# Aleph-Alpha/magma

Measured on NVIDIA H100. Metric: image-caption samples/sec (fwd+bwd), higher is better.
Workload: dtype bf16

## Files before the change

magma_b200/csrc/gemm.cu:

```cuda
#include <mutex>
#include <stdlib.h>

#include "gemm_common.cuh"

namespace mb200 {

template <int BN, bool A_MN, bool B_MN>
__global__ void __launch_bounds__(kThreads, 1)
gemm_wgmma_kernel(const __grid_constant__ CUtensorMap tmA, const __grid_constant__ CUtensorMap tmB,
                  const __grid_constant__ GemmKernelParams p) {
  using C_ = Cfg<BN>;
  constexpr int kStages = C_::kStages;

  extern __shared__ uint8_t smem_raw[];
  uint8_t* smem = reinterpret_cast<uint8_t*>((reinterpret_cast<uintptr_t>(smem_raw) + 1023) & ~uintptr_t(1023));
  uint8_t* smem_a = smem;
  uint8_t* smem_b = smem + kStages * C_::kABytes;
  float* epi_stage = reinterpret_cast<float*>(smem + kStages * C_::kStageBytes);
  uint64_t* full_bar = reinterpret_cast<uint64_t*>(smem + kStages * C_::kStageBytes + kEpiBytes);
  uint64_t* empty_bar = full_bar + kStages;

  const int wg = threadIdx.x >> 7;
  const int num_kb = (p.K + BK - 1) / BK;
  const int items = p.total_tiles * p.split_k;

  pdl_trigger();
  if (threadIdx.x == 0) {
    tma_prefetch_desc(&tmA);
    tma_prefetch_desc(&tmB);
    for (int s = 0; s < kStages; ++s) {
      mbar_init(&full_bar[s], 1);
      mbar_init(&empty_bar[s], 2);
    }
    mbar_fence_init();
  }
  __syncthreads();
  pdl_wait();

  if (wg == 0) {
    setmaxnreg_dec<40>();
    if (threadIdx.x == 0) {
      int stage = 0;
      uint32_t phase = 0;
      for (int w = blockIdx.x; w < items; w += gridDim.x) {
        const int t = w / p.split_k, ks = w - t * p.split_k;
        const int kb0 = ks * p.kb_per_split, kb1 = min(num_kb, kb0 + p.kb_per_split);
        const int tpb = p.tiles_m * p.tiles_n;
        const int z = t / tpb;
        const int r = t - z * tpb;
        const int m_blk = r % p.tiles_m;
        const int n_blk = r / p.tiles_m;
        const int z0 = z % p.nb0, z1 = z / p.nb0;
        for (int kb = kb0; kb < kb1; ++kb) {
          mbar_wait(&empty_bar[stage], phase ^ 1);
          mbar_expect_tx(&full_bar[stage], (uint32_t)C_::kStageBytes);
          uint8_t* sa = smem_a + stage * C_::kABytes;
          uint8_t* sb = smem_b + stage * C_::kBBytes;
          const int kc = kb * BK;
          if constexpr (A_MN) {
#pragma unroll
            for (int i = 0; i < BM / 64; ++i)
              tma_load_4d(sa + i * 8192, &tmA, &full_bar[stage], m_blk * BM + i * 64, kc, z0, z1);
          } else {
            tma_load_4d(sa, &tmA, &full_bar[stage], kc, m_blk * BM, z0, z1);
          }
          if constexpr (B_MN) {
#pragma unroll
            for (int i = 0; i < BN / 64; ++i)
              tma_load_4d(sb + i * 8192, &tmB, &full_bar[stage], n_blk * BN + i * 64, kc, z0, z1);
          } else {
            tma_load_4d(sb, &tmB, &full_bar[stage], kc, n_blk * BN, z0, z1);
          }
          if (++stage == kStages) {
            stage = 0;
            phase ^= 1;
          }
        }
      }
    }
  } else {
    setmaxnreg_inc<232>();
    const int cw = wg - 1;
    const bool leader = (threadIdx.x & 127) == 0;
    constexpr uint32_t b_lbo = B_MN ? 8192u : 0u;
    constexpr uint32_t a_kadv = A_MN ? 2048u : 32u, b_kadv = B_MN ? 2048u : 32u;
    const uint32_t a_off = (uint32_t)cw * 8192u;
    int stage = 0;
    uint32_t phase = 0;
    float acc[BN / 2];
    for (int w = blockIdx.x; w < items; w += gridDim.x) {
      const int t = w / p.split_k, ks = w - t * p.split_k;
      const int kb0 = ks * p.kb_per_split, kb1 = min(num_kb, kb0 + p.kb_per_split);
      const int tpb = p.tiles_m * p.tiles_n;
      const int z = t / tpb;
      const int r = t - z * tpb;
      const int m_blk = r % p.tiles_m;
      const int n_blk = r / p.tiles_m;
      const int z0 = z % p.nb0, z1 = z / p.nb0;
      int prev = -1;
      for (int kb = kb0; kb < kb1; ++kb) {
        mbar_wait(&full_bar[stage], phase);
        const uint32_t sa = smem_u32(smem_a + stage * C_::kABytes) + a_off;
        const uint32_t sb = smem_u32(smem_b + stage * C_::kBBytes);
        wgmma_fence();
#pragma unroll
        for (int k = 0; k < BK / WG_K; ++k) {
          const uint64_t da = make_smem_desc(sa + k * a_kadv, 0u, 1024);
          const uint64_t db = make_smem_desc(sb + k * b_kadv, b_lbo, 1024);
          wgmma_bf16<BN, A_MN ? 1 : 0, B_MN ? 1 : 0>(acc, da, db, (kb > kb0 || k > 0) ? 1u : 0u);
        }
        wgmma_commit();
        wgmma_wait<1>();
        if (prev >= 0 && leader) mbar_arrive(&empty_bar[prev]);
        prev = stage;
        if (++stage == kStages) {
          stage = 0;
          phase ^= 1;
        }
      }
      wgmma_wait<0>();
      if (prev >= 0 && leader) mbar_arrive(&empty_bar[prev]);
      const long long boff = (long long)z0 * p.c_bs0 + (long long)z1 * p.c_bs1;
      epi_tile<BN>(p, acc, epi_stage + cw * 64 * kEpiCols, 1 + cw, boff, m_blk * BM + cw * 64, n_blk * BN, ks);
    }
  }
}

__global__ void splitk_finalize_kernel(const GemmKernelParams p) {
  pdl_trigger();
  pdl_wait();
  const int ncol4 = (p.N + 3) >> 2;
  const long long total = (long long)p.M * ncol4;
  for (long long i = blockIdx.x * (long long)blockDim.x + threadIdx.x; i < total; i += (long long)gridDim.x * blockDim.x) {
    const int row = (int)(i / ncol4);
    const int col = (int)(i - (long long)row * ncol4) * 4;
    float v[4] = {0.f, 0.f, 0.f, 0.f};
    for (int ks = 0; ks < p.split_k; ++ks) {
      const float4 w4 = *reinterpret_cast<const float4*>(p.splitk_ws + ((long long)ks * p.M + row) * p.ld_ws + col);
      v[0] += w4.x;
      v[1] += w4.y;
      v[2] += w4.z;
      v[3] += w4.w;
    }
    epi_store4(p, 0, row, col, v);
  }
}

typedef CUresult (*PFN_encodeTiled)(CUtensorMap*, CUtensorMapDataType, cuuint32_t, void*, const cuuint64_t*,
                                    const cuuint64_t*, const cuuint32_t*, const cuuint32_t*, CUtensorMapInterleave,
                                    CUtensorMapSwizzle, CUtensorMapL2promotion, CUtensorMapFloatOOBfill);

static PFN_encodeTiled get_encode_fn() {
  static PFN_encodeTiled fn = nullptr;
  static std::once_flag once;
  std::call_once(once, [] {
    void* p = nullptr;
    cudaDriverEntryPointQueryResult qres;
    if (cudaGetDriverEntryPoint("cuTensorMapEncodeTiled", &p, cudaEnableDefault, &qres) == cudaSuccess &&
        qres == cudaDriverEntryPointSuccess)
      fn = reinterpret_cast<PFN_encodeTiled>(p);
  });
  return fn;
}

int make_operand_map(CUtensorMap* out, const mb200_operand& op, int rows, int K, int nb0, int nb1,
                            int box_rows) {
  PFN_encodeTiled enc = get_encode_fn();
  MB_REQUIRE(enc != nullptr, MB200_E_CUDA, "cuTensorMapEncodeTiled entry point unavailable");
  MB_REQUIRE((reinterpret_cast<uintptr_t>(op.ptr) & 15) == 0, MB200_E_ALIGN, "gemm operand pointer not 16B aligned");
  MB_REQUIRE(op.ld % 8 == 0, MB200_E_ALIGN, "gemm operand ld (%lld) must be a multiple of 8 elements",
             (long long)op.ld);
  MB_REQUIRE((nb0 == 1 || op.bs0 % 8 == 0) && (nb1 == 1 || op.bs1 % 8 == 0), MB200_E_ALIGN,
             "gemm operand batch strides must be multiples of 8 elements");
  cuuint64_t dims[4];
  cuuint64_t strides[3];
  cuuint32_t box[4];
  cuuint32_t estr[4] = {1, 1, 1, 1};
  if (!op.mn_major) {
    dims[0] = (cuuint64_t)K;
    dims[1] = (cuuint64_t)rows;
    box[0] = BK;
    box[1] = (cuuint32_t)box_rows;
  } else {
    dims[0] = (cuuint64_t)rows;
    dims[1] = (cuuint64_t)K;
    box[0] = 64;
    box[1] = BK;
  }
  dims[2] = (cuuint64_t)nb0;
  dims[3] = (cuuint64_t)nb1;
  box[2] = 1;
  box[3] = 1;
  strides[0] = (cuuint64_t)op.ld * 2;
  strides[1] = (cuuint64_t)(nb0 > 1 ? op.bs0 : op.ld) * 2;
  strides[2] = (cuuint64_t)(nb1 > 1 ? op.bs1 : op.ld) * 2;
  CUresult r = enc(out, CU_TENSOR_MAP_DATA_TYPE_BFLOAT16, 4, const_cast<void*>(op.ptr), dims, strides, box, estr,
                   CU_TENSOR_MAP_INTERLEAVE_NONE, CU_TENSOR_MAP_SWIZZLE_128B, CU_TENSOR_MAP_L2_PROMOTION_L2_256B,
                   CU_TENSOR_MAP_FLOAT_OOB_FILL_NONE);
  MB_REQUIRE(r == CUDA_SUCCESS, MB200_E_CUDA,
             "cuTensorMapEncodeTiled failed (%d): dims=(%llu,%llu,%llu,%llu) strides=(%llu,%llu,%llu) box=(%u,%u)",
             (int)r, (unsigned long long)dims[0], (unsigned long long)dims[1], (unsigned long long)dims[2],
             (unsigned long long)dims[3], (unsigned long long)strides[0], (unsigned long long)strides[1],
             (unsigned long long)strides[2], box[0], box[1]);
  return 0;
}

template <int BN, bool A_MN, bool B_MN>
static int launch_gemm(const CUtensorMap& tmA, const CUtensorMap& tmB, const GemmKernelParams& kp,
                       cudaStream_t stream) {
  auto kern = gemm_wgmma_kernel<BN, A_MN, B_MN>;
  static bool attr_set = false;
  if (!attr_set) {
    MB_CUDA(cudaFuncSetAttribute(kern, cudaFuncAttributeMaxDynamicSharedMemorySize, Cfg<BN>::kSmemBytes));
    attr_set = true;
  }
  const long long items = (long long)kp.total_tiles * kp.split_k;
  int grid = items < gemm_sms() ? (int)items : gemm_sms();
  {
    const double nb = (double)kp.total_tiles / ((double)kp.tiles_m * kp.tiles_n);
    const double flops = 2.0 * kp.M * (double)kp.N * kp.K * nb;
    const double bytes = nb * (2.0 * ((double)kp.M * kp.K + (double)kp.N * kp.K) + (kp.c_f32 ? 4.0 : 2.0) * kp.M * kp.N);
    GemmProfScope prof(stream, flops, bytes);
    MB_CUDA(launch_pdl(kern, dim3(grid), dim3(kThreads), Cfg<BN>::kSmemBytes, stream, tmA, tmB, kp));
  }
  count_launch();
  MB_CUDA(cudaGetLastError());
  return 0;
}

template <int BN>
static int dispatch_major(bool a_mn, bool b_mn, const CUtensorMap& tmA, const CUtensorMap& tmB,
                          const GemmKernelParams& kp, cudaStream_t s) {
  if (!a_mn && !b_mn) return launch_gemm<BN, false, false>(tmA, tmB, kp, s);
  if (!a_mn && b_mn) return launch_gemm<BN, false, true>(tmA, tmB, kp, s);
  if (a_mn && !b_mn) return launch_gemm<BN, true, false>(tmA, tmB, kp, s);
  return launch_gemm<BN, true, true>(tmA, tmB, kp, s);
}

static int dispatch_bn(int bn, bool a_mn, bool b_mn, const CUtensorMap& tmA, const CUtensorMap& tmB,
                       const GemmKernelParams& kp, cudaStream_t s) {
  switch (bn) {
    case 64: return dispatch_major<64>(a_mn, b_mn, tmA, tmB, kp, s);
    case 128: return dispatch_major<128>(a_mn, b_mn, tmA, tmB, kp, s);
    default: return dispatch_major<256>(a_mn, b_mn, tmA, tmB, kp, s);
  }
}

static int pick_bn(int M, int N, int batches) {
  if (N <= 64) return 64;
  const int tiles_m = (M + BM - 1) / BM;
  const int sms = num_sms();
  double best = 1e300;
  int best_bn = 256;
  const int cands[3] = {256, 128, 64};
  const double tile_cost[3] = {1.0, 0.55, 0.3};
  for (int i = 0; i < 3; ++i) {
    const int bn = cands[i];
    if (bn > 64 && N <= bn / 2) continue;
    const long long t = (long long)tiles_m * ((N + bn - 1) / bn) * batches;
    const long long waves = (t + sms - 1) / sms;
    const double cost = (double)waves * tile_cost[i];
    if (cost < best - 1e-12) {
      best = cost;
      best_bn = bn;
    }
  }
  return best_bn;
}

struct SmallPlan {
  int bn, split;
};
static SmallPlan plan_small_m(int N, int K, int M, size_t ws_bytes) {
  const int sms = num_sms();
  const int num_kb = (K + BK - 1) / BK;
  const double kHbmRate = 3.35e12, kItem = 4e-6, kFinalize = 4e-6;
  SmallPlan best{64, 1};
  double best_t = 1e300;
  const int cands[3] = {256, 128, 64};
  for (int i = 0; i < 3; ++i) {
    const int bn = cands[i];
    if (bn > 64 && N <= bn / 2) continue;
    const int tiles = (N + bn - 1) / bn;
    for (int split = 1; split <= 16; ++split) {
      if (split > 1) {
        if (num_kb / split < 8) break;
        if ((size_t)split * M * ((N + 3) / 4 * 4) * sizeof(float) > ws_bytes) break;
      }
      const int kb_per = (num_kb + split - 1) / split;
      const int eff_split = (num_kb + kb_per - 1) / kb_per;
      const long long items = (long long)tiles * eff_split;
      const long long waves = (items + sms - 1) / sms;
      const double active = (double)(items < sms ? items : sms);
      const double sm_rate = bn == 64 ? 40e9 : 50e9;
      const double rate = sm_rate < kHbmRate / active ? sm_rate : kHbmRate / active;
      const double t = kItem + waves * ((double)kb_per * bn * BK * 2 / rate) + (eff_split > 1 ? kFinalize : 0.0);
      if (t < best_t - 1e-12) {
        best_t = t;
        best = SmallPlan{bn, eff_split};
      }
    }
  }
  return best;
}

int gemm_impl(const mb200_gemm_args* a, cudaStream_t stream) {
  MB_REQUIRE(a != nullptr, MB200_E_ARG, "null gemm args");
  MB_REQUIRE(a->M > 0 && a->N > 0 && a->K > 0 && a->nb0 > 0 && a->nb1 > 0, MB200_E_SHAPE,
             "gemm: bad shape M=%d N=%d K=%d nb=(%d,%d)", a->M, a->N, a->K, a->nb0, a->nb1);
  MB_REQUIRE(a->c_dtype == MB200_BF16 || a->c_dtype == MB200_F32, MB200_E_DTYPE, "gemm: bad c_dtype %d", a->c_dtype);
  MB_REQUIRE(!(a->accumulate && a->c_dtype != MB200_F32), MB200_E_DTYPE, "gemm: accumulate needs f32 output");
  MB_REQUIRE(!(a->dact && !a->aux_in), MB200_E_ARG, "gemm: dact needs aux_in");
  const int celt = a->c_dtype == MB200_F32 ? 4 : 8;
  MB_REQUIRE((reinterpret_cast<uintptr_t>(a->C) & 15) == 0 && a->ldc % celt == 0, MB200_E_ALIGN,
             "gemm: C must be 16B aligned with ldc multiple of %d", celt);
  MB_REQUIRE((a->nb0 == 1 || a->c_bs0 % celt == 0) && (a->nb1 == 1 || a->c_bs1 % celt == 0), MB200_E_ALIGN,
             "gemm: C batch strides must be multiples of %d elements", celt);
  if (a->res1 || a->res2) MB_REQUIRE(a->ld_res % 8 == 0, MB200_E_ALIGN, "gemm: ld_res must be a multiple of 8");
  if (a->aux_in || a->aux_out)
    MB_REQUIRE(a->ldc % 8 == 0, MB200_E_ALIGN, "gemm: aux tensors share ldc, which must be a multiple of 8");
  int rc = check_arch();
  if (rc) return rc;

  int bn = a->force_bn ? a->force_bn : pick_bn(a->M, a->N, a->nb0 * a->nb1);
  MB_REQUIRE(bn == 64 || bn == 128 || bn == 256, MB200_E_ARG, "gemm: force_bn must be 64, 128 or 256");

  CUtensorMap tmA, tmB;
  const bool small_m = a->M <= 32 && a->A.mn_major == 0 && a->nb0 * a->nb1 == 1 && a->c_dtype == MB200_BF16;
  int plan_split = 1;
  if (small_m && !a->force_bn) {
    const SmallPlan pl = plan_small_m(a->N, a->K, a->M, a->splitk_ws ? (size_t)a->splitk_ws_bytes : 0);
    bn = pl.bn;
    plan_split = pl.split;
  }
  rc = make_operand_map(&tmA, a->A, a->M, a->K, a->nb0, a->nb1, BM);
  if (rc) return rc;

  GemmKernelParams kp;
  memset(&kp, 0, sizeof(kp));
  kp.M = a->M;
  kp.N = a->N;
  kp.K = a->K;
  kp.nb0 = a->nb0;
  kp.tiles_m = (a->M + BM - 1) / BM;
  kp.C = a->C;
  kp.ldc = a->ldc;
  kp.c_bs0 = a->c_bs0;
  kp.c_bs1 = a->c_bs1;
  kp.alpha = a->alpha;
  kp.act = a->act;
  kp.dact = a->dact;
  kp.accumulate = a->accumulate;
  kp.bias = reinterpret_cast<const bf16*>(a->bias);
  kp.aux_out = reinterpret_cast<bf16*>(a->aux_out);
  kp.aux_in = reinterpret_cast<const bf16*>(a->aux_in);
  kp.res1 = reinterpret_cast<const bf16*>(a->res1);
  kp.res2 = reinterpret_cast<const bf16*>(a->res2);
  kp.ld_res = a->ld_res;
  kp.epi_kind = EK_GENERIC;
  kp.c_f32 = a->c_dtype == MB200_F32 ? 1 : 0;
  kp.rope_tab = reinterpret_cast<const float2*>(a->rope_tab);
  kp.rope_mode = a->rope_tab ? a->rope_mode : 0;
  kp.rope_S = a->rope_S;
  kp.rope_hd = a->rope_hd;
  kp.rope_rot = a->rope_rot;
  kp.rope_ncols = a->rope_ncols;
  if (kp.rope_mode != 0)
    MB_REQUIRE(a->rope_S > 0 && a->rope_hd > 0 && a->rope_rot % 4 == 0 && a->rope_rot <= a->rope_hd &&
                   a->rope_hd % 4 == 0 && a->rope_ncols % 4 == 0,
               MB200_E_ARG, "gemm: bad rope epilogue parameters");

  const bool amn = a->A.mn_major != 0, bmn = a->B.mn_major != 0;
  kp.split_k = 1;
  kp.kb_per_split = (a->K + BK - 1) / BK;
  const bool split_mid = !small_m && a->splitk_ws && a->M <= 128 && a->nb0 * a->nb1 == 1 && a->K >= 8192 &&
                         a->N <= 8192 && !a->force_bn;
  const int bn_few = a->N >= 256 ? 256 : (a->N > 64 ? 128 : 64);
  const int tiles_m = kp.tiles_m;
  const bool split_few = !small_m && !split_mid && a->splitk_ws && a->M > 128 && a->nb0 * a->nb1 == 1 &&
                         a->K >= 2048 && !a->force_bn && 2 * tiles_m * ((a->N + bn_few - 1) / bn_few) <= num_sms();
  if (plan_split > 1 || split_mid || split_few) {
    const int bn_s = small_m ? bn : bn_few;
    const int tiles = (a->N + bn_s - 1) / bn_s;
    const int num_kb = (a->K + BK - 1) / BK;
    int split = plan_split;
    if (split_mid || split_few) {
      split = num_sms() / (tiles * tiles_m);
      if (split > num_kb / 4) split = num_kb / 4;
    }
    const long long ld_ws = (a->N + 3) / 4 * 4;
    while (split > 1 && (size_t)split * a->M * ld_ws * sizeof(float) > (size_t)a->splitk_ws_bytes) --split;
    if (split > 1) {
      const int kb_per = (num_kb + split - 1) / split;
      split = (num_kb + kb_per - 1) / kb_per;
      bn = bn_s;
      rc = make_operand_map(&tmB, a->B, a->N, a->K, a->nb0, a->nb1, bn);
      if (rc) return rc;
      kp.tiles_n = tiles;
      kp.total_tiles = tiles_m * tiles;
      kp.split_k = split;
      kp.kb_per_split = kb_per;
      kp.splitk_ws = reinterpret_cast<float*>(a->splitk_ws);
      kp.ld_ws = ld_ws;
      GemmKernelParams kg = kp;
      kg.epi_kind = EK_SPLITK;
      rc = dispatch_bn(bn, amn, bmn, tmA, tmB, kg, stream);
      if (rc) return rc;
      const long long n4 = (long long)a->M * ((a->N + 3) / 4);
      const int fgrid = (int)((n4 + 255) / 256 > 2048 ? 2048 : (n4 + 255) / 256);
      kp.alpha = 1.f;
      MB_CUDA(launch_pdl(splitk_finalize_kernel, dim3(fgrid), dim3(256), 0, stream, kp));
      count_launch();
      return 0;
    }
  }
  rc = make_operand_map(&tmB, a->B, a->N, a->K, a->nb0, a->nb1, bn);
  if (rc) return rc;
  kp.tiles_n = (a->N + bn - 1) / bn;
  kp.total_tiles = tiles_m * kp.tiles_n * a->nb0 * a->nb1;
  return dispatch_bn(bn, amn, bmn, tmA, tmB, kp, stream);
}

}

extern "C" int mb200_gemm(const mb200_gemm_args* args, void* stream) {
  return mb200::gemm_impl(args, reinterpret_cast<cudaStream_t>(stream));
}
```

magma_b200/csrc/gemm_common.cuh:

```cuda
#pragma once
#include "common.cuh"

namespace mb200 {

static constexpr int BM = 128;
static constexpr int BK = 64;
static constexpr int WG_K = 16;
static constexpr int kThreads = 384;
static constexpr int kEpiCols = 64;
static constexpr int kEpiBytes = BM * kEpiCols * 4;
static constexpr int kSmemBudget = 192 * 1024;

template <int BN>
struct Cfg {
  static constexpr int kABytes = BM * BK * 2;
  static constexpr int kBBytes = BN * BK * 2;
  static constexpr int kStageBytes = kABytes + kBBytes;
  static constexpr int kStagesRaw = kSmemBudget / kStageBytes;
  static constexpr int kStages = kStagesRaw > 8 ? 8 : kStagesRaw;
  static constexpr int kSmemBytes = kStages * kStageBytes + kEpiBytes + 1024  + 256 ;
  static_assert(kSmemBytes <= 227 * 1024, "GEMM shared memory exceeds the sm_90 per-block limit");
};

struct GemmKernelParams {
  int M, N, K;
  int nb0;
  int tiles_m, tiles_n, total_tiles;
  void* C;
  long long ldc, c_bs0, c_bs1;
  float alpha;
  int act, dact, accumulate;
  const bf16* bias;
  bf16* aux_out;
  const bf16* aux_in;
  const bf16* res1;
  const bf16* res2;
  long long ld_res;
  const float2* rope_tab;
  int rope_mode;
  int rope_S, rope_hd, rope_rot, rope_ncols;
  int epi_kind;
  int c_f32;
  int split_k, kb_per_split;
  float* splitk_ws;
  long long ld_ws;
};

__device__ __forceinline__ float2 bf16x2_to_f32(uint32_t u) {
  return __bfloat1622float2(*reinterpret_cast<const __nv_bfloat162*>(&u));
}
__device__ __forceinline__ uint32_t f32x2_to_bf16(float a, float b) {
  __nv_bfloat162 h = __floats2bfloat162_rn(a, b);
  return *reinterpret_cast<uint32_t*>(&h);
}

__device__ __forceinline__ void ld_bf16x4(const bf16* src, int n, float (&v)[4]) {
  if (n == 4 && (reinterpret_cast<uintptr_t>(src) & 7) == 0) {
    uint32_t u0, u1;
    asm volatile("ld.global.nc.v2.u32 {%0, %1}, [%2];" : "=r"(u0), "=r"(u1) : "l"(src));
    const float2 a = bf16x2_to_f32(u0), b = bf16x2_to_f32(u1);
    v[0] = a.x;
    v[1] = a.y;
    v[2] = b.x;
    v[3] = b.y;
  } else {
#pragma unroll
    for (int e = 0; e < 4; ++e) v[e] = e < n ? __bfloat162float(src[e]) : 0.f;
  }
}
__device__ __forceinline__ void st_bf16x4(bf16* dst, int n, const float (&v)[4]) {
  if (n == 4 && (reinterpret_cast<uintptr_t>(dst) & 7) == 0) {
    *reinterpret_cast<uint2*>(dst) = make_uint2(f32x2_to_bf16(v[0], v[1]), f32x2_to_bf16(v[2], v[3]));
  } else {
#pragma unroll
    for (int e = 0; e < 4; ++e)
      if (e < n) dst[e] = __float2bfloat16(v[e]);
  }
}

__device__ __forceinline__ void named_bar_sync(int id, int nthreads) {
  asm volatile("bar.sync %0, %1;" ::"r"(id), "r"(nthreads) : "memory");
}

enum { EK_GENERIC = 0, EK_SPLITK };

__device__ __forceinline__ void epi_store4(const GemmKernelParams& p, long long boff, int row, int col, float (&v)[4]) {
  const int n = min(4, p.N - col);
  if (p.bias) {
    float b[4];
    ld_bf16x4(p.bias + col, n, b);
#pragma unroll
    for (int e = 0; e < 4; ++e) v[e] += b[e];
  }
  if (p.rope_mode != 0 && col < p.rope_ncols) {
    const int dim = col % p.rope_hd;
    if (dim < p.rope_rot) {
      const float2* tp = p.rope_tab + (long long)(row % p.rope_S) * (p.rope_rot >> 1) + (dim >> 1);
      const float2 cs0 = __ldg(tp), cs1 = __ldg(tp + 1);
      const float sg = p.rope_mode > 0 ? 1.f : -1.f;
      const float a0 = v[0], a1 = v[1], a2 = v[2], a3 = v[3];
      v[0] = a0 * cs0.x - a1 * cs0.y * sg;
      v[1] = a1 * cs0.x + a0 * cs0.y * sg;
      v[2] = a2 * cs1.x - a3 * cs1.y * sg;
      v[3] = a3 * cs1.x + a2 * cs1.y * sg;
    }
  }
  const long long coff = boff + (long long)row * p.ldc + col;
  if (p.aux_out) st_bf16x4(p.aux_out + coff, n, v);
#pragma unroll
  for (int e = 0; e < 4; ++e) {
    if (p.act == MB200_ACT_GELU_NEW) v[e] = gelu_new_f(v[e]);
    else if (p.act == MB200_ACT_QUICK_GELU) v[e] = quick_gelu_f(v[e]);
    else if (p.act == MB200_ACT_RELU) v[e] = fmaxf(v[e], 0.f);
  }
  if (p.dact) {
    float a[4];
    ld_bf16x4(p.aux_in + coff, n, a);
#pragma unroll
    for (int e = 0; e < 4; ++e) v[e] = p.dact == MB200_DACT_GELU_NEW ? v[e] * gelu_new_grad_f(a[e]) : (a[e] > 0.f ? v[e] : 0.f);
  }
  const long long roff = boff + (long long)row * p.ld_res + col;
  if (p.res1) {
    float r[4];
    ld_bf16x4(p.res1 + roff, n, r);
#pragma unroll
    for (int e = 0; e < 4; ++e) v[e] += r[e];
  }
  if (p.res2) {
    float r[4];
    ld_bf16x4(p.res2 + roff, n, r);
#pragma unroll
    for (int e = 0; e < 4; ++e) v[e] += r[e];
  }
  if (p.act == MB200_ACT_RELU_POST) {
#pragma unroll
    for (int e = 0; e < 4; ++e) v[e] = fmaxf(v[e], 0.f);
  }
  if (p.c_f32) {
    float* dst = reinterpret_cast<float*>(p.C) + coff;
    if (n == 4) {
      float4 o = make_float4(v[0], v[1], v[2], v[3]);
      if (p.accumulate) {
        const float4 old = *reinterpret_cast<const float4*>(dst);
        o.x += old.x;
        o.y += old.y;
        o.z += old.z;
        o.w += old.w;
      }
      *reinterpret_cast<float4*>(dst) = o;
    } else {
#pragma unroll
      for (int e = 0; e < 4; ++e)
        if (e < n) dst[e] = p.accumulate ? dst[e] + v[e] : v[e];
    }
  } else {
    st_bf16x4(reinterpret_cast<bf16*>(p.C) + coff, n, v);
  }
}

template <int BN>
__device__ __forceinline__ void epi_tile(const GemmKernelParams& p, const float (&acc)[BN / 2], float* stage,
                                         int bar_id, long long boff, int row0, int col0, int ks) {
  const int wt = threadIdx.x & 127;
  const int fr = (wt >> 5) * 16 + ((wt & 31) >> 2);
  const int fq = wt & 3;
  const int pr = wt >> 4, pc = wt & 15;
  const int nch = min(BN / kEpiCols, (p.N - col0 + kEpiCols - 1) / kEpiCols);
#pragma unroll 1
  for (int ch = 0; ch < nch; ++ch) {
#pragma unroll
    for (int c = 0; c < BN / kEpiCols; ++c) {
      if (c != ch) continue;
#pragma unroll
      for (int jj = 0; jj < 8; ++jj) {
        const int j = c * 8 + jj;
#pragma unroll
        for (int h = 0; h < 2; ++h) {
          const int r = fr + 8 * h;
          const int q = (2 * jj + (fq >> 1)) ^ ((r & 3) << 1);
          *reinterpret_cast<float2*>(stage + r * kEpiCols + q * 4 + 2 * (fq & 1)) =
              make_float2(acc[4 * j + 2 * h], acc[4 * j + 2 * h + 1]);
        }
      }
    }
    named_bar_sync(bar_id, 128);
    const int col = col0 + ch * kEpiCols + pc * 4;
#pragma unroll 1
    for (int i = 0; i < 64 / 8; ++i) {
      const int r = pr + 8 * i;
      const int row = row0 + r;
      if (row >= p.M || col >= p.N) continue;
      const float4 s = *reinterpret_cast<const float4*>(stage + r * kEpiCols + ((pc ^ ((r & 3) << 1)) * 4));
      float v[4] = {s.x * p.alpha, s.y * p.alpha, s.z * p.alpha, s.w * p.alpha};
      if (p.epi_kind == EK_SPLITK) {
        *reinterpret_cast<float4*>(p.splitk_ws + ((long long)ks * p.M + row) * p.ld_ws + col) =
            make_float4(v[0], v[1], v[2], v[3]);
        continue;
      }
      epi_store4(p, boff, row, col, v);
    }
    named_bar_sync(bar_id, 128);
  }
}

int make_operand_map(CUtensorMap* out, const mb200_operand& op, int rows, int K, int nb0, int nb1, int box_rows);

}
```

Before: 129.4.

## Add ping-pong 64x256 consumer schedule and widen epilogue stores to 8 columns

Adds a ping-pong variant of the WGMMA GEMM in which each consumer warpgroup owns a whole 64x256 tile and alternates tiles with the other warpgroup. Named barriers order their mainloops so one group's epilogue overlaps the other's MMA, and a ring-advance helper skips the other group's stages. The tile picker now weighs this variant against the cooperative ones. Separately, the epilogue processes 8 columns per thread (two float4 smem reads, wider bf16 stores) to cut per-element loop overhead. This adds template instantiations and barrier complexity, and smaller M tiles raise B-operand traffic.

```diff
diff --git a/magma_b200/csrc/gemm.cu b/magma_b200/csrc/gemm.cu
--- a/magma_b200/csrc/gemm.cu
+++ b/magma_b200/csrc/gemm.cu
@@ -5,12 +5,25 @@
 
 namespace mb200 {
 
-template <int BN, bool A_MN, bool B_MN>
+__device__ __forceinline__ int item_kblocks(const GemmKernelParams& p, int num_kb, int w) {
+  const int kb0 = (w % p.split_k) * p.kb_per_split;
+  return min(num_kb, kb0 + p.kb_per_split) - kb0;
+}
+
+template <int kStages>
+__device__ __forceinline__ void ring_advance(int& stage, uint32_t& phase, int n) {
+  const int s = stage + n;
+  stage = s % kStages;
+  phase ^= (uint32_t)(s / kStages) & 1u;
+}
+
+template <int BN, bool PP, bool A_MN, bool B_MN>
 __global__ void __launch_bounds__(kThreads, 1)
 gemm_wgmma_kernel(const __grid_constant__ CUtensorMap tmA, const __grid_constant__ CUtensorMap tmB,
                   const __grid_constant__ GemmKernelParams p) {
-  using C_ = Cfg<BN>;
+  using C_ = Cfg<BN, PP>;
   constexpr int kStages = C_::kStages;
+  constexpr int TM = C_::kBM;
 
   extern __shared__ uint8_t smem_raw[];
   uint8_t* smem = reinterpret_cast<uint8_t*>((reinterpret_cast<uintptr_t>(smem_raw) + 1023) & ~uintptr_t(1023));
@@ -30,7 +43,7 @@
     tma_prefetch_desc(&tmB);
     for (int s = 0; s < kStages; ++s) {
       mbar_init(&full_bar[s], 1);
-      mbar_init(&empty_bar[s], 2);
+      mbar_init(&empty_bar[s], PP ? 1 : 2);
     }
     mbar_fence_init();
   }
@@ -59,10 +72,10 @@
           const int kc = kb * BK;
           if constexpr (A_MN) {
 #pragma unroll
-            for (int i = 0; i < BM / 64; ++i)
-              tma_load_4d(sa + i * 8192, &tmA, &full_bar[stage], m_blk * BM + i * 64, kc, z0, z1);
+            for (int i = 0; i < TM / 64; ++i)
+              tma_load_4d(sa + i * 8192, &tmA, &full_bar[stage], m_blk * TM + i * 64, kc, z0, z1);
           } else {
-            tma_load_4d(sa, &tmA, &full_bar[stage], kc, m_blk * BM, z0, z1);
+            tma_load_4d(sa, &tmA, &full_bar[stage], kc, m_blk * TM, z0, z1);
           }
           if constexpr (B_MN) {
 #pragma unroll
@@ -84,11 +97,14 @@
     const bool leader = (threadIdx.x & 127) == 0;
     constexpr uint32_t b_lbo = B_MN ? 8192u : 0u;
     constexpr uint32_t a_kadv = A_MN ? 2048u : 32u, b_kadv = B_MN ? 2048u : 32u;
-    const uint32_t a_off = (uint32_t)cw * 8192u;
     int stage = 0;
     uint32_t phase = 0;
     float acc[BN / 2];
-    for (int w = blockIdx.x; w < items; w += gridDim.x) {
+    const int i0 = PP ? cw : 0, di = PP ? 2 : 1;
+    if (PP && cw == 1 && blockIdx.x < items) ring_advance<kStages>(stage, phase, item_kblocks(p, num_kb, blockIdx.x));
+    for (int i = i0;; i += di) {
+      const int w = blockIdx.x + i * gridDim.x;
+      if (w >= items) break;
       const int t = w / p.split_k, ks = w - t * p.split_k;
       const int kb0 = ks * p.kb_per_split, kb1 = min(num_kb, kb0 + p.kb_per_split);
       const int tpb = p.tiles_m * p.tiles_n;
@@ -97,6 +113,9 @@
       const int m_blk = r % p.tiles_m;
       const int n_blk = r / p.tiles_m;
       const int z0 = z % p.nb0, z1 = z / p.nb0;
+      const int w_next = w + gridDim.x;
+      if (PP && i > 0) named_bar_sync(3 + cw, 256);
+      const uint32_t a_off = PP ? 0u : (uint32_t)cw * 8192u;
       int prev = -1;
       for (int kb = kb0; kb < kb1; ++kb) {
         mbar_wait(&full_bar[stage], phase);
@@ -118,10 +137,15 @@
           phase ^= 1;
         }
       }
+      if (PP && w_next < items) {
+        named_bar_arrive(3 + (cw ^ 1), 256);
+        ring_advance<kStages>(stage, phase, item_kblocks(p, num_kb, w_next));
+      }
       wgmma_wait<0>();
       if (prev >= 0 && leader) mbar_arrive(&empty_bar[prev]);
       const long long boff = (long long)z0 * p.c_bs0 + (long long)z1 * p.c_bs1;
-      epi_tile<BN>(p, acc, epi_stage + cw * 64 * kEpiCols, 1 + cw, boff, m_blk * BM + cw * 64, n_blk * BN, ks);
+      const int row0 = m_blk * TM + (PP ? 0 : cw * 64);
+      epi_tile<BN>(p, acc, epi_stage + cw * 64 * kEpiCols, 1 + cw, boff, row0, n_blk * BN, ks);
     }
   }
 }
@@ -142,7 +166,7 @@
       v[2] += w4.z;
       v[3] += w4.w;
     }
-    epi_store4(p, 0, row, col, v);
+    epi_store<4>(p, 0, row, col, v);
   }
 }
 
@@ -205,13 +229,13 @@
   return 0;
 }
 
-template <int BN, bool A_MN, bool B_MN>
+template <int BN, bool PP, bool A_MN, bool B_MN>
 static int launch_gemm(const CUtensorMap& tmA, const CUtensorMap& tmB, const GemmKernelParams& kp,
                        cudaStream_t stream) {
-  auto kern = gemm_wgmma_kernel<BN, A_MN, B_MN>;
+  auto kern = gemm_wgmma_kernel<BN, PP, A_MN, B_MN>;
   static bool attr_set = false;
   if (!attr_set) {
-    MB_CUDA(cudaFuncSetAttribute(kern, cudaFuncAttributeMaxDynamicSharedMemorySize, Cfg<BN>::kSmemBytes));
+    MB_CUDA(cudaFuncSetAttribute(kern, cudaFuncAttributeMaxDynamicSharedMemorySize, Cfg<BN, PP>::kSmemBytes));
     attr_set = true;
   }
   const long long items = (long long)kp.total_tiles * kp.split_k;
@@ -221,51 +245,55 @@
     const double flops = 2.0 * kp.M * (double)kp.N * kp.K * nb;
     const double bytes = nb * (2.0 * ((double)kp.M * kp.K + (double)kp.N * kp.K) + (kp.c_f32 ? 4.0 : 2.0) * kp.M * kp.N);
     GemmProfScope prof(stream, flops, bytes);
-    MB_CUDA(launch_pdl(kern, dim3(grid), dim3(kThreads), Cfg<BN>::kSmemBytes, stream, tmA, tmB, kp));
+    MB_CUDA(launch_pdl(kern, dim3(grid), dim3(kThreads), Cfg<BN, PP>::kSmemBytes, stream, tmA, tmB, kp));
   }
   count_launch();
   MB_CUDA(cudaGetLastError());
   return 0;
 }
 
-template <int BN>
+template <int BN, bool PP>
 static int dispatch_major(bool a_mn, bool b_mn, const CUtensorMap& tmA, const CUtensorMap& tmB,
                           const GemmKernelParams& kp, cudaStream_t s) {
-  if (!a_mn && !b_mn) return launch_gemm<BN, false, false>(tmA, tmB, kp, s);
-  if (!a_mn && b_mn) return launch_gemm<BN, false, true>(tmA, tmB, kp, s);
-  if (a_mn && !b_mn) return launch_gemm<BN, true, false>(tmA, tmB, kp, s);
-  return launch_gemm<BN, true, true>(tmA, tmB, kp, s);
-}
-
-static int dispatch_bn(int bn, bool a_mn, bool b_mn, const CUtensorMap& tmA, const CUtensorMap& tmB,
+  if (!a_mn && !b_mn) return launch_gemm<BN, PP, false, false>(tmA, tmB, kp, s);
+  if (!a_mn && b_mn) return launch_gemm<BN, PP, false, true>(tmA, tmB, kp, s);
+  if (a_mn && !b_mn) return launch_gemm<BN, PP, true, false>(tmA, tmB, kp, s);
+  return launch_gemm<BN, PP, true, true>(tmA, tmB, kp, s);
+}
+
+static int dispatch_bn(int bn, bool pp, bool a_mn, bool b_mn, const CUtensorMap& tmA, const CUtensorMap& tmB,
                        const GemmKernelParams& kp, cudaStream_t s) {
+  if (pp) return dispatch_major<256, true>(a_mn, b_mn, tmA, tmB, kp, s);
   switch (bn) {
-    case 64: return dispatch_major<64>(a_mn, b_mn, tmA, tmB, kp, s);
-    case 128: return dispatch_major<128>(a_mn, b_mn, tmA, tmB, kp, s);
-    default: return dispatch_major<256>(a_mn, b_mn, tmA, tmB, kp, s);
-  }
-}
-
-static int pick_bn(int M, int N, int batches) {
-  if (N <= 64) return 64;
-  const int tiles_m = (M + BM - 1) / BM;
+    case 64: return dispatch_major<64, false>(a_mn, b_mn, tmA, tmB, kp, s);
+    case 128: return dispatch_major<128, false>(a_mn, b_mn, tmA, tmB, kp, s);
+    default: return dispatch_major<256, false>(a_mn, b_mn, tmA, tmB, kp, s);
+  }
+}
+
+struct TilePlan {
+  int bn;
+  bool pp;
+};
+static TilePlan pick_tile(int M, int N, int batches) {
+  if (N <= 64) return TilePlan{64, false};
   const int sms = num_sms();
   double best = 1e300;
-  int best_bn = 256;
-  const int cands[3] = {256, 128, 64};
-  const double tile_cost[3] = {1.0, 0.55, 0.3};
-  for (int i = 0; i < 3; ++i) {
-    const int bn = cands[i];
+  TilePlan plan{256, false};
+  const TilePlan cands[4] = {{256, false}, {256, true}, {128, false}, {64, false}};
+  const double tile_cost[4] = {1.0, 0.55, 0.55, 0.3};
+  for (int i = 0; i < 4; ++i) {
+    const int bn = cands[i].bn, bm = cands[i].pp ? Cfg<256, true>::kBM : BM;
     if (bn > 64 && N <= bn / 2) continue;
-    const long long t = (long long)tiles_m * ((N + bn - 1) / bn) * batches;
+    const long long t = (long long)((M + bm - 1) / bm) * ((N + bn - 1) / bn) * batches;
     const long long waves = (t + sms - 1) / sms;
     const double cost = (double)waves * tile_cost[i];
     if (cost < best - 1e-12) {
       best = cost;
-      best_bn = bn;
-    }
-  }
-  return best_bn;
+      plan = cands[i];
+    }
+  }
+  return plan;
 }
 
 struct SmallPlan {
@@ -322,7 +350,8 @@
   int rc = check_arch();
   if (rc) return rc;
 
-  int bn = a->force_bn ? a->force_bn : pick_bn(a->M, a->N, a->nb0 * a->nb1);
+  const TilePlan plan = a->force_bn ? TilePlan{a->force_bn, false} : pick_tile(a->M, a->N, a->nb0 * a->nb1);
+  int bn = plan.bn;
   MB_REQUIRE(bn == 64 || bn == 128 || bn == 256, MB200_E_ARG, "gemm: force_bn must be 64, 128 or 256");
 
   CUtensorMap tmA, tmB;
@@ -404,7 +433,7 @@
       kp.ld_ws = ld_ws;
       GemmKernelParams kg = kp;
       kg.epi_kind = EK_SPLITK;
-      rc = dispatch_bn(bn, amn, bmn, tmA, tmB, kg, stream);
+      rc = dispatch_bn(bn, false, amn, bmn, tmA, tmB, kg, stream);
       if (rc) return rc;
       const long long n4 = (long long)a->M * ((a->N + 3) / 4);
       const int fgrid = (int)((n4 + 255) / 256 > 2048 ? 2048 : (n4 + 255) / 256);
@@ -414,11 +443,17 @@
       return 0;
     }
   }
+  const bool pp = plan.pp && !small_m;
+  if (pp) {
+    kp.tiles_m = (a->M + Cfg<256, true>::kBM - 1) / Cfg<256, true>::kBM;
+    rc = make_operand_map(&tmA, a->A, a->M, a->K, a->nb0, a->nb1, Cfg<256, true>::kBM);
+    if (rc) return rc;
+  }
   rc = make_operand_map(&tmB, a->B, a->N, a->K, a->nb0, a->nb1, bn);
   if (rc) return rc;
   kp.tiles_n = (a->N + bn - 1) / bn;
-  kp.total_tiles = tiles_m * kp.tiles_n * a->nb0 * a->nb1;
-  return dispatch_bn(bn, amn, bmn, tmA, tmB, kp, stream);
+  kp.total_tiles = kp.tiles_m * kp.tiles_n * a->nb0 * a->nb1;
+  return dispatch_bn(bn, pp, amn, bmn, tmA, tmB, kp, stream);
 }
 
 }
diff --git a/magma_b200/csrc/gemm_common.cuh b/magma_b200/csrc/gemm_common.cuh
--- a/magma_b200/csrc/gemm_common.cuh
+++ b/magma_b200/csrc/gemm_common.cuh
@@ -8,12 +8,14 @@
 static constexpr int WG_K = 16;
 static constexpr int kThreads = 384;
 static constexpr int kEpiCols = 64;
-static constexpr int kEpiBytes = BM * kEpiCols * 4;
+static constexpr int kEpiBytes = 2 * 64 * kEpiCols * 4;
 static constexpr int kSmemBudget = 192 * 1024;
 
-template <int BN>
+template <int BN, bool PP>
 struct Cfg {
-  static constexpr int kABytes = BM * BK * 2;
+  static_assert(!PP || BN == 256, "the ping-pong tile is 64 x 256");
+  static constexpr int kBM = PP ? 64 : BM;
+  static constexpr int kABytes = kBM * BK * 2;
   static constexpr int kBBytes = BN * BK * 2;
   static constexpr int kStageBytes = kABytes + kBBytes;
   static constexpr int kStagesRaw = kSmemBudget / kStageBytes;
@@ -81,80 +83,117 @@
 __device__ __forceinline__ void named_bar_sync(int id, int nthreads) {
   asm volatile("bar.sync %0, %1;" ::"r"(id), "r"(nthreads) : "memory");
 }
+__device__ __forceinline__ void named_bar_arrive(int id, int nthreads) {
+  asm volatile("bar.arrive %0, %1;" ::"r"(id), "r"(nthreads) : "memory");
+}
 
 enum { EK_GENERIC = 0, EK_SPLITK };
 
-__device__ __forceinline__ void epi_store4(const GemmKernelParams& p, long long boff, int row, int col, float (&v)[4]) {
-  const int n = min(4, p.N - col);
+template <int W>
+__device__ __forceinline__ void epi_store(const GemmKernelParams& p, long long boff, int row, int col, float (&v)[W]) {
+  static_assert(W == 4 || W == 8, "epi_store: W must be 4 or 8");
+  constexpr int G = W / 4;
+  int ng[G];
+#pragma unroll
+  for (int g = 0; g < G; ++g) ng[g] = max(0, min(4, p.N - col - 4 * g));
+  auto grp = [&](int g) -> float(&)[4] { return *reinterpret_cast<float(*)[4]>(v + 4 * g); };
   if (p.bias) {
-    float b[4];
-    ld_bf16x4(p.bias + col, n, b);
-#pragma unroll
-    for (int e = 0; e < 4; ++e) v[e] += b[e];
-  }
-  if (p.rope_mode != 0 && col < p.rope_ncols) {
-    const int dim = col % p.rope_hd;
-    if (dim < p.rope_rot) {
-      const float2* tp = p.rope_tab + (long long)(row % p.rope_S) * (p.rope_rot >> 1) + (dim >> 1);
-      const float2 cs0 = __ldg(tp), cs1 = __ldg(tp + 1);
-      const float sg = p.rope_mode > 0 ? 1.f : -1.f;
-      const float a0 = v[0], a1 = v[1], a2 = v[2], a3 = v[3];
-      v[0] = a0 * cs0.x - a1 * cs0.y * sg;
-      v[1] = a1 * cs0.x + a0 * cs0.y * sg;
-      v[2] = a2 * cs1.x - a3 * cs1.y * sg;
-      v[3] = a3 * cs1.x + a2 * cs1.y * sg;
+#pragma unroll
+    for (int g = 0; g < G; ++g) {
+      float b[4];
+      ld_bf16x4(p.bias + col + 4 * g, ng[g], b);
+#pragma unroll
+      for (int e = 0; e < 4; ++e) v[4 * g + e] += b[e];
+    }
+  }
+  if (p.rope_mode != 0) {
+#pragma unroll
+    for (int g = 0; g < G; ++g) {
+      const int cg = col + 4 * g;
+      if (cg >= p.rope_ncols) continue;
+      const int dim = cg % p.rope_hd;
+      if (dim < p.rope_rot) {
+        const float2* tp = p.rope_tab + (long long)(row % p.rope_S) * (p.rope_rot >> 1) + (dim >> 1);
+        const float2 cs0 = __ldg(tp), cs1 = __ldg(tp + 1);
+        const float sg = p.rope_mode > 0 ? 1.f : -1.f;
+        float* u = v + 4 * g;
+        const float a0 = u[0], a1 = u[1], a2 = u[2], a3 = u[3];
+        u[0] = a0 * cs0.x - a1 * cs0.y * sg;
+        u[1] = a1 * cs0.x + a0 * cs0.y * sg;
+        u[2] = a2 * cs1.x - a3 * cs1.y * sg;
+        u[3] = a3 * cs1.x + a2 * cs1.y * sg;
+      }
     }
   }
   const long long coff = boff + (long long)row * p.ldc + col;
-  if (p.aux_out) st_bf16x4(p.aux_out + coff, n, v);
-#pragma unroll
-  for (int e = 0; e < 4; ++e) {
+  if (p.aux_out) {
+#pragma unroll
+    for (int g = 0; g < G; ++g) st_bf16x4(p.aux_out + coff + 4 * g, ng[g], grp(g));
+  }
+#pragma unroll
+  for (int e = 0; e < W; ++e) {
     if (p.act == MB200_ACT_GELU_NEW) v[e] = gelu_new_f(v[e]);
     else if (p.act == MB200_ACT_QUICK_GELU) v[e] = quick_gelu_f(v[e]);
     else if (p.act == MB200_ACT_RELU) v[e] = fmaxf(v[e], 0.f);
   }
   if (p.dact) {
-    float a[4];
-    ld_bf16x4(p.aux_in + coff, n, a);
-#pragma unroll
-    for (int e = 0; e < 4; ++e) v[e] = p.dact == MB200_DACT_GELU_NEW ? v[e] * gelu_new_grad_f(a[e]) : (a[e] > 0.f ? v[e] : 0.f);
+#pragma unroll
+    for (int g = 0; g < G; ++g) {
+      float a[4];
+      ld_bf16x4(p.aux_in + coff + 4 * g, ng[g], a);
+#pragma unroll
+      for (int e = 0; e < 4; ++e)
+        v[4 * g + e] = p.dact == MB200_DACT_GELU_NEW ? v[4 * g + e] * gelu_new_grad_f(a[e])
+                                                     : (a[e] > 0.f ? v[4 * g + e] : 0.f);
+    }
   }
   const long long roff = boff + (long long)row * p.ld_res + col;
   if (p.res1) {
-    float r[4];
-    ld_bf16x4(p.res1 + roff, n, r);
-#pragma unroll
-    for (int e = 0; e < 4; ++e) v[e] += r[e];
+#pragma unroll
+    for (int g = 0; g < G; ++g) {
+      float r[4];
+      ld_bf16x4(p.res1 + roff + 4 * g, ng[g], r);
+#pragma unroll
+      for (int e = 0; e < 4; ++e) v[4 * g + e] += r[e];
+    }
   }
   if (p.res2) {
-    float r[4];
-    ld_bf16x4(p.res2 + roff, n, r);
-#pragma unroll
-    for (int e = 0; e < 4; ++e) v[e] += r[e];
+#pragma unroll
+    for (int g = 0; g < G; ++g) {
+      float r[4];
+      ld_bf16x4(p.res2 + roff + 4 * g, ng[g], r);
+#pragma unroll
+      for (int e = 0; e < 4; ++e) v[4 * g + e] += r[e];
+    }
   }
   if (p.act == MB200_ACT_RELU_POST) {
 #pragma unroll
-    for (int e = 0; e < 4; ++e) v[e] = fmaxf(v[e], 0.f);
+    for (int e = 0; e < W; ++e) v[e] = fmaxf(v[e], 0.f);
   }
   if (p.c_f32) {
-    float* dst = reinterpret_cast<float*>(p.C) + coff;
-    if (n == 4) {
-      float4 o = make_float4(v[0], v[1], v[2], v[3]);
-      if (p.accumulate) {
-        const float4 old = *reinterpret_cast<const float4*>(dst);
-        o.x += old.x;
-        o.y += old.y;
-        o.z += old.z;
-        o.w += old.w;
-      }
-      *reinterpret_cast<float4*>(dst) = o;
-    } else {
-#pragma unroll
-      for (int e = 0; e < 4; ++e)
-        if (e < n) dst[e] = p.accumulate ? dst[e] + v[e] : v[e];
+#pragma unroll
+    for (int g = 0; g < G; ++g) {
+      float* dst = reinterpret_cast<float*>(p.C) + coff + 4 * g;
+      const float* u = v + 4 * g;
+      if (ng[g] == 4) {
+        float4 o = make_float4(u[0], u[1], u[2], u[3]);
+        if (p.accumulate) {
+          const float4 old = *reinterpret_cast<const float4*>(dst);
+          o.x += old.x;
+          o.y += old.y;
+          o.z += old.z;
+          o.w += old.w;
+        }
+        *reinterpret_cast<float4*>(dst) = o;
+      } else {
+#pragma unroll
+        for (int e = 0; e < 4; ++e)
+          if (e < ng[g]) dst[e] = p.accumulate ? dst[e] + u[e] : u[e];
+      }
     }
   } else {
-    st_bf16x4(reinterpret_cast<bf16*>(p.C) + coff, n, v);
+#pragma unroll
+    for (int g = 0; g < G; ++g) st_bf16x4(reinterpret_cast<bf16*>(p.C) + coff + 4 * g, ng[g], grp(g));
   }
 }
 
@@ -164,7 +203,7 @@
   const int wt = threadIdx.x & 127;
   const int fr = (wt >> 5) * 16 + ((wt & 31) >> 2);
   const int fq = wt & 3;
-  const int pr = wt >> 4, pc = wt & 15;
+  const int pr = wt >> 3, pc = wt & 7;
   const int nch = min(BN / kEpiCols, (p.N - col0 + kEpiCols - 1) / kEpiCols);
 #pragma unroll 1
   for (int ch = 0; ch < nch; ++ch) {
@@ -184,20 +223,23 @@
       }
     }
     named_bar_sync(bar_id, 128);
-    const int col = col0 + ch * kEpiCols + pc * 4;
+    const int col = col0 + ch * kEpiCols + pc * 8;
 #pragma unroll 1
-    for (int i = 0; i < 64 / 8; ++i) {
-      const int r = pr + 8 * i;
+    for (int i = 0; i < 64 / 16; ++i) {
+      const int r = pr + 16 * i;
       const int row = row0 + r;
       if (row >= p.M || col >= p.N) continue;
-      const float4 s = *reinterpret_cast<const float4*>(stage + r * kEpiCols + ((pc ^ ((r & 3) << 1)) * 4));
-      float v[4] = {s.x * p.alpha, s.y * p.alpha, s.z * p.alpha, s.w * p.alpha};
+      const float4 s0 = *reinterpret_cast<const float4*>(stage + r * kEpiCols + (((2 * pc) ^ ((r & 3) << 1)) * 4));
+      const float4 s1 = *reinterpret_cast<const float4*>(stage + r * kEpiCols + (((2 * pc + 1) ^ ((r & 3) << 1)) * 4));
+      float v[8] = {s0.x * p.alpha, s0.y * p.alpha, s0.z * p.alpha, s0.w * p.alpha,
+                    s1.x * p.alpha, s1.y * p.alpha, s1.z * p.alpha, s1.w * p.alpha};
       if (p.epi_kind == EK_SPLITK) {
-        *reinterpret_cast<float4*>(p.splitk_ws + ((long long)ks * p.M + row) * p.ld_ws + col) =
-            make_float4(v[0], v[1], v[2], v[3]);
+        float* ws = p.splitk_ws + ((long long)ks * p.M + row) * p.ld_ws + col;
+        *reinterpret_cast<float4*>(ws) = make_float4(v[0], v[1], v[2], v[3]);
+        if (col + 4 < p.N) *reinterpret_cast<float4*>(ws + 4) = make_float4(v[4], v[5], v[6], v[7]);
         continue;
       }
-      epi_store4(p, boff, row, col, v);
+      epi_store<8>(p, boff, row, col, v);
     }
     named_bar_sync(bar_id, 128);
   }
```

Measured after the change: 137.9 (median of 6 runs). 1.07x the previous value.
